# lucabaldesi/srsRAN

Hardware: AMD Instinct MI355X
Metric: PDSCH decoded Mbps + code-blocks/sec, 20 MHz TM4 QAM256, 1/2/4/8 GPU (higher is better)
Workload: dtype fp32+int16; 1 GPU; srslte_ue_dl chain from time-domain I/Q: 2048 subframes/GPU/batch, 20 MHz (100 PRB), TM4 2x2 spatial multiplexing, 2 codewords QAM256 TBS 97896 (C=16, K=6144), MMSE+CSI, max 10 half-its with CRC early stop, 40 dB crossed 2x2 channel, every subframe distinct (GPU eNodeB generator, keyed by global subframe index); 3 PHY worker threads (own ue_dl / stream / softbuffers each) decode alternate batches,; subframes_per_gpu_batch=2048, code_blocks_per_gpu_batch=65536, workers_per_gpu=3, parallelism=dp1

## Files before the change

### include/srsran_amd/dlsch.h

```cpp
#ifndef SRSRAN_AMD_DLSCH_H
#define SRSRAN_AMD_DLSCH_H

#include <stddef.h>
#include <stdint.h>

#ifdef __cplusplus
extern "C" {
#endif

typedef struct mi355_softbuffer_pool mi355_softbuffer_pool_t;

int  mi355_softbuffer_pool_create(mi355_softbuffer_pool_t** p, uint32_t nof_sb, uint32_t max_cb, int device);
void mi355_softbuffer_pool_destroy(mi355_softbuffer_pool_t* p);
int mi355_softbuffer_reset(mi355_softbuffer_pool_t* p, uint32_t sb, void* stream);
int mi355_softbuffer_reset_tbs(mi355_softbuffer_pool_t* p, uint32_t sb, uint32_t tbs, void* stream);
int mi355_softbuffer_reset_cb(mi355_softbuffer_pool_t* p, uint32_t sb, uint32_t nof_cb, void* stream);
int mi355_softbuffer_reset_all(mi355_softbuffer_pool_t* p, void* stream);
int mi355_softbuffer_reset_range(mi355_softbuffer_pool_t* p, uint32_t first, uint32_t n, void* stream);
int mi355_softbuffer_reset_tbs_batch(mi355_softbuffer_pool_t* p, const uint32_t* sbs, const uint32_t* tbs, uint32_t n,
                                     void* stream);
int mi355_softbuffer_pool_buffer(mi355_softbuffer_pool_t* p, int16_t** buf, uint32_t* stride, uint32_t* max_cb);
int mi355_softbuffer_pool_materialize(mi355_softbuffer_pool_t* p, uint32_t first, uint32_t n, void* stream);

int mi355_softbuffer_pool_data(mi355_softbuffer_pool_t* p, uint8_t** data, uint32_t* stride, uint32_t* nof_sb);
// ... 6 lines not shown
  uint32_t Qm;
  uint32_t rv;
  uint32_t softbuffer;
  uint64_t e_offset;
  uint64_t data_offset;
} mi355_dlsch_tb_t;

typedef struct mi355_dlsch mi355_dlsch_t;

int  mi355_dlsch_create(mi355_dlsch_t** q, int device);
void mi355_dlsch_destroy(mi355_dlsch_t* q);
int mi355_dlsch_set_max_iterations(mi355_dlsch_t* q, uint32_t max_iterations);
void mi355_dlsch_set_profiling(mi355_dlsch_t* q, int enable);

int mi355_dlsch_set_latency_path(int max_cbs);
int mi355_dlsch_latency_profile(int enable, uint64_t* out);
int  mi355_dlsch_kernel_stats(mi355_dlsch_t* q, double* ms, uint32_t* launches);

int mi355_dlsch_decode_dev(mi355_dlsch_t*           q,
                           mi355_softbuffer_pool_t* pool,
                           const int16_t*           d_e_bits,
                           const mi355_dlsch_tb_t*  tbs,
                           uint32_t                 ntb,
                           uint8_t*                 d_data,
                           int32_t*                 ret,
                           float*                   avg_iterations,
                           void*                    stream);

int mi355_dlsch_decode8_dev(mi355_dlsch_t* q, mi355_softbuffer_pool_t* pool, const int8_t* d_e_bits,
                            const mi355_dlsch_tb_t* tbs, uint32_t ntb, uint8_t* d_data, int32_t* ret,
// ... 7 lines not shown
```

### srsran_amd/csrc/dlsch_internal.h

```cpp
#pragma once
#include <hip/hip_runtime.h>
#include <stdint.h>

#define SB_STRIDE 18600
#define SB_DATA 768
#define SB_CONV8 10240
#define SB_ROWMASK 18544
#define SB_ROWMASK_WORDS 12

namespace mi355 {

struct CbDesc {
  uint32_t tb, cb, C;
  uint32_t rlen;
  uint32_t rp, n_e;
  uint32_t rv;
  uint32_t slot;
  uint64_t e_off;
  uint64_t data_off;
};

struct TbDesc {
  uint32_t tbs, C, C1, K1, K2, slot0, invalid;
  uint32_t Qm, nof_e_bits, rv;
  uint32_t cb_base[2];
  uint64_t e_off;
  uint64_t data_off;
  const uint32_t* crc_scale;
};

struct CrcTable {
  uint32_t t[256];
  uint32_t pw[24];
  uint32_t poly;
};

CrcTable make_crc_table(uint32_t poly);

constexpr uint16_t RM_NONE = 0xffff;

struct DlschRmArgs {
  const CbDesc*   desc;
  int             ncb;
  uint32_t        N;
  uint32_t        buflen;
  const uint16_t* inv[4];
  const int16_t*  e;
  int16_t*        sb;
  size_t          sb_stride;
  const uint8_t*  sb_crc;
  uint8_t*        fresh;
  uint32_t        fold2;
// ... 16 lines not shown
struct DlschCheckArgs {
  const CbDesc*  desc;
  int            ncb;
  uint32_t       K, h, max_its;
  const uint8_t* dec;
  size_t         dec_stride;
  uint8_t*       data;
  uint8_t*       done;
  const uint32_t* remaining;
  uint32_t*      next;
  uint32_t*      its;
  uint8_t*        sb_crc;
  const CrcTable* crc24a;
  const CrcTable* crc24b;
  const uint32_t* scale;
};

struct DlschTbArgs {
  const TbDesc* tb;
  int           ntb;
  uint8_t*      data;
  uint8_t*      sb_crc;
  uint8_t*      sb_data;
  int32_t*        ret;
  const CrcTable* crc24a;
  CbDesc*   desc;
  uint32_t* slot;
  uint32_t* its;
  uint8_t*  done;
  uint32_t* running;
  float*    avg;
};

struct DlschResetArgs {
  uint8_t* fresh;
  uint8_t* sb_crc;
  size_t   slot0, ncb;
  size_t   ncrc;
};

hipError_t dlsch_launch_rm(const DlschRmArgs& a, hipStream_t s);
hipError_t dlsch_launch_reset_list(const uint2* list, uint32_t n, uint32_t max_cb, uint8_t* fresh, uint8_t* cb_crc,
                                   hipStream_t s);
hipError_t dlsch_launch_check(const DlschCheckArgs& a, hipStream_t s);
hipError_t dlsch_launch_prologue(const DlschTbArgs& a, hipStream_t s);
hipError_t dlsch_launch_epilogue(const DlschTbArgs& a, hipStream_t s);
// ... 8 lines not shown
```

### srsran_amd/csrc/dlsch_kernels.hip

```cpp
#include <hip/hip_runtime.h>
#include <stdint.h>

#include "crc_device.h"
#include "dlsch_internal.h"
#include "rm_image.h"

namespace mi355 {

constexpr uint32_t RM_LDS     = 3 * 6144 + 12;
constexpr uint32_t RM_THREADS = 512;
constexpr int      RM_Q       = (3 * (6144 + 32) + 12 + 8 * RM_THREADS - 1) / (8 * RM_THREADS);
constexpr int      RM_EQ      = (RM_LDS + 8 * RM_THREADS - 1) / (8 * RM_THREADS);
#ifndef RM_CPB_N
#define RM_CPB_N 1
#endif
constexpr int      RM_CPB     = RM_CPB_N;

__device__ __forceinline__ uint32_t add_pairs(uint32_t a, uint32_t b)
{
  return ((a + b) & 0xffffu) | (((a >> 16) + (b >> 16)) << 16);
}

__device__ __forceinline__ uint4 ld_quad(const uint32_t* p, uint32_t q, uint32_t lim, bool al16, uint32_t fill)
{
// ... 174 lines not shown
    bool           todo  = false;
    if (lane < 3) data[tb.tbs / 8 + lane] = 0;
    for (uint32_t c = lane; c < tb.C; c += 64) {
      const uint32_t K    = c < tb.C1 ? tb.K1 : tb.K2;
      const uint32_t rlen = tb.C == 1 ? K : K - 24;
      uint32_t       rp = c * n_e, n_e2 = n_e;
      if (c > tb.C - gamma) {
        n_e2 = n_e + tb.Qm;
        rp   = (tb.C - gamma) * n_e + (c - (tb.C - gamma)) * n_e2;
      }
      const uint32_t g    = c < tb.C1 ? tb.cb_base[0] + c : tb.cb_base[1] + (c - tb.C1);
      const uint32_t slot = tb.slot0 + c;
      a.desc[g]           = CbDesc{(uint32_t)t, c, tb.C, rlen, rp, n_e2, tb.rv, slot, tb.e_off, tb.data_off};
      a.slot[g]           = slot;
      a.its[g]            = 0;
      const bool prior    = a.sb_crc[slot] != 0;
      a.done[g]           = prior ? 3 : 0;
      todo |= !prior;
    }
    if (todo) todo_any = 1;
    for (uint32_t c = 0; c < tb.C; c++) {
      const uint32_t slot = tb.slot0 + c;
      if (!a.sb_crc[slot]) continue;
      const uint32_t K    = c < tb.C1 ? tb.K1 : tb.K2;
      const uint32_t rlen = tb.C == 1 ? K : K - 24;
      const uint32_t o    = c * rlen / 8;
      for (uint32_t i = lane; i < rlen / 8; i += 64) data[o + i] = a.sb_data[(size_t)slot * 768 + i];
    }
  }
  __syncthreads();
  if (threadIdx.x == 0 && todo_any) flag_set(a.running);
}

__global__ __launch_bounds__(256) void dlsch_tb_epilogue(DlschTbArgs a)
{
  const int t   = blockIdx.x;
  const int tid = threadIdx.x;
  if (t >= a.ntb) return;
  __shared__ uint32_t t4[4][256];
  t4[0][tid] = a.crc24a->t[tid];
  __syncthreads();
  const TbDesc& tb = a.tb[t];
  if (tb.crc_scale) {
#pragma unroll
    for (int k = 1; k < 4; k++) {
      t4[k][tid] = crc24_step_table(t4[k - 1][tid], t4[0]);
      __syncthreads();
    }
  }
  if (tid == 0) {
    double sum = 0.0;
    for (uint32_t c = 0; c < tb.C; c++) sum += a.its[c < tb.C1 ? tb.cb_base[0] + c : tb.cb_base[1] + (c - tb.C1)];
    a.avg[t] = tb.C ? (float)(sum / tb.C) : 0.f;
  }
  if (tb.C == 0) {
    if (tid == 0) a.ret[t] = tb.invalid ? -2 : 0;
    return;
  }
  bool ok = true;
  for (uint32_t c = 0; c < tb.C; c++) ok &= a.sb_crc[tb.slot0 + c] != 0;
  uint8_t* data = a.data + tb.data_off;
  if (!ok) {
    for (uint32_t c = 0; c < tb.C; c++) {
      const uint32_t slot = tb.slot0 + c;
      if (!a.sb_crc[slot]) continue;
      const uint32_t K    = c < tb.C1 ? tb.K1 : tb.K2;
      const uint32_t rlen = tb.C == 1 ? K : K - 24;
      for (uint32_t i = tid; i < rlen / 8; i += blockDim.x) a.sb_data[(size_t)slot * 768 + i] = data[c * rlen / 8 + i];
    }
    if (tid == 0) a.ret[t] = -1;
    return;
  }
  const uint32_t par_rx = tb.crc_scale ? block_crc24_scaled4(data, tb.tbs / 8, t4, a.crc24a->poly, tb.crc_scale)
                                        : block_crc24(data, tb.tbs / 8, t4[0], *a.crc24a);
  if (tid == 0) {
    const uint32_t par_tx = ((uint32_t)data[tb.tbs / 8] << 16) | ((uint32_t)data[tb.tbs / 8 + 1] << 8) |
                            (uint32_t)data[tb.tbs / 8 + 2];
    a.ret[t] = (par_rx == par_tx && par_rx) ? 0 : -1;
  }
}

__global__ __launch_bounds__(256) void dlsch_sb_reset(DlschResetArgs a)
{
  const size_t g = (size_t)blockIdx.x * blockDim.x + threadIdx.x;
  if (g < a.ncb) a.fresh[a.slot0 + g] = 1;
  if (g < (a.ncrc ? a.ncrc : a.ncb)) a.sb_crc[a.slot0 + g] = 0;
}

__global__ __launch_bounds__(256) void dlsch_sb_reset_list(const uint2* list, uint32_t n, uint32_t max_cb, uint8_t* fresh,
                                                           uint8_t* cb_crc)
// ... 93 lines not shown
hipError_t dlsch_launch_check(const DlschCheckArgs& a, hipStream_t s)
{
  hipLaunchKernelGGL(dlsch_cb_check, dim3((unsigned)((a.ncb + 15) / 16)), dim3(1024), 0, s, a);
  return hipGetLastError();
}

hipError_t dlsch_launch_prologue(const DlschTbArgs& a, hipStream_t s)
{
  hipLaunchKernelGGL(dlsch_tb_prologue, dim3((unsigned)((a.ntb + 3) / 4)), dim3(256), 0, s, a);
  return hipGetLastError();
}

hipError_t dlsch_launch_epilogue(const DlschTbArgs& a, hipStream_t s)
{
  if (a.ntb <= 0) return hipSuccess;
  hipLaunchKernelGGL(dlsch_tb_epilogue, dim3((unsigned)a.ntb), dim3(256), 0, s, a);
  return hipGetLastError();
}

hipError_t dlsch_launch_reset(const DlschResetArgs& a, hipStream_t s)
{
  const size_t n = a.ncb > a.ncrc ? a.ncb : a.ncrc;
  if (!n) return hipSuccess;
  hipLaunchKernelGGL(dlsch_sb_reset, dim3((unsigned)((n + 255) / 256)), dim3(256), 0, s, a);
  return hipGetLastError();
}

}
```

### srsran_amd/csrc/dlsch_runtime.cpp

```cpp
#include <hip/hip_runtime.h>

#include <algorithm>
#include <chrono>
#include <stdlib.h>
#include <map>
#include <mutex>
#include <stdio.h>
#include <string.h>
#include <vector>

#include "../../include/srsran_amd/dlsch.h"
#include "../../include/srsran_amd/tdec.h"
#include "dlsch_internal.h"
#include "host_staging.h"
#include "tdec8_internal.h"
#include "rm_image.h"
#include "rm_tables.h"
#include "runtime_internal.h"
#include "tdec_internal.h"

using namespace mi355;

#define CHECK_HIP(x)                                                                                                   \
  do {                                                                                                                 \
// ... 48 lines not shown
struct mi355_dlsch {
  int                                    device = 0;
  hipStream_t                            own    = nullptr;
  uint32_t                               max_its = 10;
  std::map<uint32_t, mi355_tdec_batch_t*> dec;
  std::map<uint64_t, uint16_t*>          rm;
  std::map<uint64_t, uint16_t*>          rm8;
  struct Compact {
    uint16_t* d;
    uint32_t  nq, qoff;
  };
  std::map<uint64_t, Compact>            rmc;
  std::map<uint32_t, mi355_tdec8_t*>     dec8;
  std::map<uint32_t, uint32_t*>          scales;
  std::map<uint32_t, uint32_t*>          tb_scales;
  CrcTable*                              crc = nullptr;
  char*      scratch[2]     = {nullptr, nullptr};
  size_t     scratch_cap[2] = {0, 0};
  std::vector<void*> retired;
  hipEvent_t done_ev[2]     = {nullptr, nullptr};
  bool       done_armed[2]  = {false, false};
  uint32_t   par            = 0;
  std::mutex mu;
  bool       prof = false;
  HostStaging stage;
  HostStaging back;
  std::atomic<uint32_t> spec_mask{1u << 1};
};

static std::atomic<int> g_lat_cbs{-1};
// ... 26 lines not shown
  }
  return MI355_SUCCESS;
}

extern "C" int mi355_dlsch_set_latency_path(int max_cbs)
{
  const int old = lat_cbs_now();
  if (max_cbs >= 0) g_lat_cbs.store(max_cbs);
  return old;
}

static bool spec_enabled()
{
  static const bool on = !getenv("MI355_TDEC_SPEC") || atoi(getenv("MI355_TDEC_SPEC")) != 0;
  return on;
}

static bool no_rowmask()
{
  static const bool off = getenv("MI355_NO_ROWMASK") && atoi(getenv("MI355_NO_ROWMASK")) != 0;
  return off;
}

static bool lat_waves4()
{
  static const bool on = getenv("MI355_LAT_WAVES") && atoi(getenv("MI355_LAT_WAVES")) == 4;
  return on;
}
static bool lat_owaves()
{
// ... 59 lines not shown
static uint32_t gf2_mulmod24_host(uint32_t a, uint32_t b, uint32_t poly)
{
  uint32_t r = 0;
  for (int i = 23; i >= 0; i--) {
    r <<= 1;
    if (r & 0x1000000u) r ^= poly;
    if ((b >> i) & 1u) r ^= a;
  }
  return r & 0xffffffu;
}

static int crc_scales(mi355_dlsch_t* q, uint32_t K, const uint32_t** out)
{
  auto it = q->scales.find(K);
  if (it == q->scales.end()) {
    std::vector<uint32_t> t(144, 0u);
    const uint32_t        nbytes = K / 8, chunk = (nbytes + 63) / 64;
    const uint32_t        polys[2] = {0x1864CFB, 0x1800063};
    auto                  xpow = [](uint32_t after, uint32_t poly) {
      uint32_t sc = 1, x8 = 1u << 8;
      for (; after; after >>= 1) {
        if (after & 1) sc = gf2_mulmod24_host(sc, x8, poly);
        x8 = gf2_mulmod24_host(x8, x8, poly);
      }
      return sc;
    };
    const uint32_t nl = std::max(1u, mi355_tdec_autoimp_get_subblocks(K) / 2), cl = nbytes / nl;
    for (int pi = 0; pi < 2; pi++) {
      for (uint32_t lane = 0; lane < 64; lane++) {
        const uint32_t b0 = std::min(nbytes, lane * chunk), b1 = std::min(nbytes, b0 + chunk);
        t[pi * 64 + lane] = xpow(nbytes - b1, polys[pi]);
      }
      for (uint32_t l = 0; l < nl && l < 8; l++) t[128 + 8 * pi + l] = xpow(nbytes - (l + 1) * cl, polys[pi]);
    }
    uint32_t* d = nullptr;
    CHECK_HIP(hipMalloc(&d, t.size() * 4));
    CHECK_HIP(hipMemcpy(d, t.data(), t.size() * 4, hipMemcpyHostToDevice));
    it = q->scales.emplace(K, d).first;
  }
  *out = it->second;
  return MI355_SUCCESS;
}

static int tb_crc_scales(mi355_dlsch_t* q, uint32_t nbytes, const uint32_t** out)
{
  auto it = q->tb_scales.find(nbytes);
  if (it == q->tb_scales.end()) {
    std::vector<uint32_t> t(256);
    const uint32_t        chunk = ((nbytes + 255) / 256 + 3) / 4 * 4, poly = 0x1864CFB;
// ... 3 lines not shown
      for (uint32_t after = nbytes - b1; after; after >>= 1) {
        if (after & 1) sc = gf2_mulmod24_host(sc, x8, poly);
        x8 = gf2_mulmod24_host(x8, x8, poly);
      }
      t[tid] = sc;
    }
    uint32_t* d = nullptr;
    CHECK_HIP(hipMalloc(&d, t.size() * 4));
    CHECK_HIP(hipMemcpy(d, t.data(), t.size() * 4, hipMemcpyHostToDevice));
    it = q->tb_scales.emplace(nbytes, d).first;
  }
  *out = it->second;
  return MI355_SUCCESS;
}

static int scratch(mi355_dlsch_t* q, uint32_t k, size_t bytes, char** p)
{
  if (bytes > q->scratch_cap[k]) {
    if (q->scratch[k]) {
      q->retired.push_back(q->scratch[k]);
      q->scratch[k]    = nullptr;
      q->done_armed[k] = false;
    }
    size_t cap = bytes + bytes / 4 + 4096;
    CHECK_HIP(hipMalloc(&q->scratch[k], cap));
    q->scratch_cap[k] = cap;
  }
  *p = q->scratch[k];
  return MI355_SUCCESS;
}
// ... 187 lines not shown
  return MI355_SUCCESS;
}

void mi355_dlsch_destroy(mi355_dlsch_t* q)
{
  if (!q) return;
  (void)hipSetDevice(q->device);
  (void)hipDeviceSynchronize();
  for (auto& kv : q->dec) mi355_tdec_batch_destroy(kv.second);
  for (auto& kv : q->rm) (void)hipFree(kv.second);
  for (auto& kv : q->rm8) (void)hipFree(kv.second);
  for (auto& kv : q->rmc) (void)hipFree(kv.second.d);
  for (auto& kv : q->dec8) mi355_tdec8_destroy(kv.second);
  for (auto& kv : q->scales) (void)hipFree(kv.second);
  for (auto& kv : q->tb_scales) (void)hipFree(kv.second);
  (void)hipFree(q->crc);
  for (void* r : q->retired) (void)hipFree(r);
  for (int k = 0; k < 2; k++) {
    (void)hipFree(q->scratch[k]);
    if (q->done_ev[k]) (void)hipEventDestroy(q->done_ev[k]);
  }
  if (q->own) (void)hipStreamDestroy(q->own);
  delete q;
}

int mi355_dlsch_set_max_iterations(mi355_dlsch_t* q, uint32_t max_iterations)
{
  if (!q || max_iterations == 0) return MI355_ERROR_INVALID_INPUTS;
  q->max_its = max_iterations;
  return MI355_SUCCESS;
// ... 116 lines not shown
      if (j >= 32 * SB_ROWMASK_WORDS || j >= K / 16) return true;
      for (uint32_t w = 0; w < 16; w++)
        if (inv[s * sl + j * 16 + w] < E) return true;
      return false;
    };
    std::vector<uint16_t> rank(nquad, 0xffff);
    std::vector<uint32_t> qlist;
    for (uint32_t qd = 0; qd < nquad; qd++) {
      if (!defined(8 * qd)) continue;
      uint32_t m = 0;
      for (uint32_t p = 0; p < 8 && 8 * qd + p < buflen; p++) m |= (uint32_t)(inv[8 * qd + p] < E) << p;
      rank[qd] = (uint16_t)qlist.size();
      qlist.push_back(qd | m << 16);
    }
    const uint32_t        off = (E + 7) / 8 * 8;
    std::vector<uint16_t> all(off + 2 * qlist.size() + 8, 0);
    for (uint32_t r = 0; r < E; r++) {
      const uint32_t pos = t[r];
      if (rank[pos / 8] == 0xffff) return MI355_ERROR;
      all[r] = (uint16_t)(8 * rank[pos / 8] + pos % 8);
    }
    memcpy(all.data() + off, qlist.data(), qlist.size() * 4);
    uint16_t* d = nullptr;
    CHECK_HIP(hipMalloc(&d, all.size() * 2));
    CHECK_HIP(hipMemcpy(d, all.data(), all.size() * 2, hipMemcpyHostToDevice));
    CHECK_HIP(hipStreamSynchronize(nullptr));
    it = q->rmc.emplace(key, mi355_dlsch::Compact{d, (uint32_t)qlist.size(), off}).first;
  }
  *tab  = it->second.d;
  *nq   = it->second.nq;
  *qoff = it->second.qoff;
  return MI355_SUCCESS;
}

mi355::SoftbufferView mi355::softbuffer_view(mi355_softbuffer_pool_t* p)
{
  return SoftbufferView{p->buf, SB_STRIDE, p->cb_crc, p->fresh, p->nof_sb, p->max_cb};
}

int mi355::dlsch_decode_dev_hook(mi355_dlsch_t* q, mi355_softbuffer_pool_t* pool, const void* d_e_bits,
                                 const mi355_dlsch_tb_t* tbs, uint32_t ntb, uint8_t* d_data, int32_t* ret,
                                 float* avg_iterations, void* stream, mi355::WaitHook hook, bool llr8,
                                 mi355::DlschPending* pend, bool after_s, bool rm_done)
{
  if (!q || !pool || !tbs || !ret || (ntb && !d_e_bits)) return MI355_ERROR_INVALID_INPUTS;
  if (ntb == 0) return MI355_SUCCESS;
  std::lock_guard<std::mutex> lock(q->mu);
  static const bool prof = getenv("MI355_HOST_PROF") != nullptr;
  auto              now  = [] { return std::chrono::steady_clock::now(); };
  const auto        t0   = now();
  CHECK_HIP(hipSetDevice(q->device));
  hipStream_t s = stream ? (hipStream_t)stream : q->own;

  std::vector<TbDesc>                        tbd(ntb);
  std::vector<std::pair<uint32_t, uint32_t>> kcount;
  std::vector<uint32_t>                      rvmask;
  std::vector<uint32_t>                      fold2;
  auto group_of = [&](uint32_t K) {
    for (uint32_t i = 0; i < kcount.size(); i++)
      if (kcount[i].first == K) return i;
    kcount.push_back({K, 0u});
    rvmask.push_back(0u);
    return (uint32_t)kcount.size() - 1;
  };
  std::vector<uint8_t> grp(2 * ntb, 0);
  uint32_t             seg_tbs = UINT32_MAX;
  CbSegm               seg{};
// ... 11 lines not shown
    if (in.softbuffer >= pool->nof_sb || in.rv > 3 || in.Qm == 0 || seg_err) {
      d.invalid = 1;
      continue;
    }
    if (in.tbs == 0 || seg.C == 0) continue;
    if (seg.F || seg.C > pool->max_cb) {
      d.invalid = 1;
      continue;
    }
    auto ok8 = [](uint32_t K) { return tdec_subblocks_8bit(K) >= 16 || K <= 400; };
    if (llr8 && ((seg.C1 && !ok8(seg.K1)) || (seg.C > seg.C1 && !ok8(seg.K2)))) {
      d.invalid = 1;
      continue;
    }
    if (int e = tb_crc_scales(q, in.tbs / 8, &d.crc_scale)) return e;
    d.C          = seg.C;
    d.C1         = seg.C1;
    d.K1         = seg.K1;
    d.K2         = seg.K2;
    d.slot0      = in.softbuffer * pool->max_cb;
    d.Qm         = in.Qm;
    d.nof_e_bits = in.nof_e_bits;
    d.rv         = in.rv;
    d.e_off      = in.e_offset;
    const uint32_t emax = in.Qm * (in.nof_e_bits / in.Qm / seg.C + 1);
    auto           fold = [&](uint32_t g, uint32_t K) {
      if (fold2.size() <= g) fold2.resize(g + 1, 0);
      fold2[g] = std::max(fold2[g], std::min(emax, 3 * K + 12) / 2);
    };
    if (seg.C1) {
// ... 16 lines not shown
  std::vector<uint32_t> goff(kcount.size());
  size_t                total_cb = 0, dec_bytes = 0;
  for (size_t g = 0; g < kcount.size(); g++) {
    goff[g] = (uint32_t)total_cb;
    total_cb += kcount[g].second;
    dec_bytes += (size_t)kcount[g].second * (kcount[g].first / 8);
  }
  for (uint32_t t = 0; t < ntb; t++) {
    if (!tbd[t].C) continue;
    tbd[t].cb_base[0] += goff[grp[2 * t]];
    tbd[t].cb_base[1] += goff[grp[2 * t + 1]];
  }

  auto rnd = [](size_t b) { return (b + 255) / 256 * 256; };
  const size_t need = rnd(ntb * sizeof(TbDesc)) + rnd(4 * (q->max_its + 1)) + rnd(total_cb * sizeof(CbDesc)) +
                      3 * rnd(total_cb * 4) + rnd(total_cb) + rnd(dec_bytes) + 2 * rnd(ntb * 4);
  const uint32_t slot = q->par;
  q->par ^= 1u;
  char* base = nullptr;
  int   r    = scratch(q, slot, need, &base);
  if (r) return r;
  char* p     = base;
  auto  carve = [&](size_t b) {
    char* c = p;
    p += rnd(b);
    return c;
  };
  auto*        d_tb    = (TbDesc*)carve(ntb * sizeof(TbDesc));
  auto*        d_run   = (uint32_t*)carve(4 * (q->max_its + 1));
  const size_t staged  = (size_t)(p - base);
  auto*        d_cb    = (CbDesc*)carve(total_cb * sizeof(CbDesc));
  auto*        d_slot  = (uint32_t*)carve(total_cb * 4);
  auto*        d_its   = (uint32_t*)carve(total_cb * 4);
  auto*        d_done  = (uint8_t*)carve(total_cb);
  auto*        d_dec   = (uint8_t*)carve(dec_bytes);
  auto*        d_ret   = (int32_t*)carve(ntb * 4);
  auto*        d_avg   = (float*)carve(ntb * 4);

  CHECK_HIP(q->stage.reserve(staged));
  q->stage.put(tbd.data(), ntb * sizeof(TbDesc));
  q->stage.zeros(4 * (q->max_its + 1));
  CHECK_HIP(q->stage.upload(base, s, false, after_s && q->done_armed[slot] ? q->done_ev[slot] : nullptr));

  DlschTbArgs ta{d_tb,  (int)ntb, d_data, pool->cb_crc, pool->data, d_ret, &q->crc[0],
                 d_cb,  d_slot,   d_its,  d_done,       d_run,      d_avg};
  CHECK_HIP(dlsch_launch_prologue(ta, s));

  struct Live {
    uint32_t            K, off, n;
    uint8_t*            dec;
    mi355_tdec_batch_t* td;
    const uint32_t*     scale;
    mi355_tdec8_t*      t8 = nullptr;
  };
  std::vector<Live> live;
  size_t            off = 0, doff = 0;
  for (size_t gi = 0; gi < kcount.size(); gi++) {
    const uint32_t K = kcount[gi].first, n = kcount[gi].second;
    if (llr8) {
      const uint32_t nsb8 = tdec_subblocks_8bit(K);
// ... 94 lines not shown
  }
  const uint32_t spec_mask = spec_enabled() ? q->spec_mask.load() : 0u;
  for (uint32_t h = 0; h < q->max_its; h++) {
    const bool spec = h + 1 == q->max_its || ((spec_mask >> h) & 1u);
    for (size_t li = 0; li < live.size(); li++) {
      auto& lv = live[li];
      if (lat[li]) continue;
      if (lv.t8) {
        T8Batch b{};
        b.in = (int8_t*)pool->buf, b.in_stride = SB_STRIDE * sizeof(int16_t), b.slot = d_slot + lv.off;
        b.done = d_done + lv.off, b.running = d_run + h, b.K = lv.K, b.ncb = lv.n;
        if ((r = tdec8_halfit_batch(lv.t8, b, h, lv.dec, lv.K / 8, s))) return r;
      }
      DlschCheckArgs ca{d_cb + lv.off, (int)lv.n, lv.K, h, q->max_its, lv.dec, lv.K / 8, d_data,
                        d_done + lv.off, d_run + h, d_run + h + 1, d_its + lv.off, pool->cb_crc, &q->crc[0], &q->crc[1],
                        lv.scale};
      bool fused = false;
      if (!lv.t8) {
        TdecRun rq{llr8 ? pool->buf + SB_CONV8 : pool->buf, SB_STRIDE, d_slot + lv.off, d_done + lv.off, d_run + h, lv.n,
                   lv.K, h, h + 1, lv.dec, lv.K / 8, s, &ca, &fused};
        rq.rowmask = !llr8 && !no_rowmask();
        bool taken = false;
        rq.spec       = spec;
        rq.spec_taken = &taken;
        if ((r = mi355_tdec_run_internal(lv.td, rq))) return r;
        if (!fused) CHECK_HIP(dlsch_launch_check(ca, s));
        if (taken && h + 1 < q->max_its) {
          TdecRun rd = rq;
          rd.remaining  = d_run + h + 1;
          rd.chk        = nullptr;
          rd.chk_fused  = nullptr;
// ... 57 lines not shown
```

### srsran_amd/csrc/pdsch_internal.h

```cpp
#pragma once
#include <hip/hip_runtime.h>
#include <stdint.h>

namespace mi355 {

constexpr uint32_t EQ_BLOCK_ITEMS = 1024;

constexpr uint32_t PDSCH_GOLD_MAX = 14u * 12u * 110u * 8u;

struct PdschJobDev {
  const float2*   y[2];
  const float2*   h[4][2];
  const uint16_t* map;
  const uint16_t* imap;
  uint32_t        g0;
  float2*         d[2];
  float*          csi[2];
  uint32_t*       cmax;
  uint32_t        cmax_stride;
  uint32_t        nof_re, nof_rx, nof_ports, nof_layers, scheme, cb;
  uint32_t        row;
  uint32_t        row_magic;
  uint32_t        h_invariant;
  uint32_t        rhob_mask;
// ... 26 lines not shown

hipError_t pdsch_launch_equalize(const PdschJobDev* jobs, uint32_t njobs, uint32_t max_units, hipStream_t s);
hipError_t pdsch_launch_scr_pack(const uint32_t* c_init, uint32_t* const* dst, uint32_t n, const uint32_t* gold,
                                 uint32_t W, hipStream_t s);
hipError_t pdsch_launch_llr(const PdschCwDev* cws, uint32_t ncw, uint32_t max_pairs, hipStream_t s);
hipError_t pdsch_launch_fused(const PdschJobDev* jobs, uint32_t njobs, uint32_t max_pairs, const uint32_t* keys,
                              uint32_t nkeys, hipStream_t s);

struct EqRmLayer {
  const uint16_t* inv[2];
  uint32_t        N[2];
  uint32_t        buflen[2];
  uint32_t        C1;
  uint32_t        slot0;
};
struct EqRmJob {
  uint32_t  C, Qm, Gp;
  EqRmLayer layer[2];
  const uint16_t* cmp[2][2];
  uint32_t        cnq[2][2], cqoff[2][2];
};
struct EqRmPool {
  int16_t*       sb;
  size_t         sb_stride;
  const uint8_t* sb_crc;
  uint8_t*       fresh;
  int            sparse;
  int            diag = 0;
  unsigned long long* prof = nullptr;
};
hipError_t pdsch_launch_eq_rm(const PdschJobDev* jobs, const EqRmJob* rj, uint32_t njobs, uint32_t max_c, uint32_t img,
                              uint32_t cimg, const uint32_t* keys, uint32_t nkeys, const EqRmPool& pool, hipStream_t s);

// ... 2 lines not shown
```

### srsran_amd/csrc/pdsch_kernels.hip

```cpp
#include <hip/hip_runtime.h>

#include <algorithm>
#include <stdint.h>

#include "pdsch_internal.h"
#include "rm_image.h"
#include "xcd.h"

namespace mi355 {

namespace {

struct cf {
  float re, im;
};
__device__ __forceinline__ cf mk(float r, float i) { return cf{r, i}; }
__device__ __forceinline__ cf operator+(cf a, cf b) { return mk(a.re + b.re, a.im + b.im); }
__device__ __forceinline__ cf operator-(cf a, cf b) { return mk(a.re - b.re, a.im - b.im); }
__device__ __forceinline__ cf operator*(cf a, cf b) { return mk(a.re * b.re - a.im * b.im, a.re * b.im + a.im * b.re); }
__device__ __forceinline__ cf operator*(cf a, float s) { return mk(a.re * s, a.im * s); }
__device__ __forceinline__ cf cj(cf a) { return mk(a.re, -a.im); }
__device__ __forceinline__ cf mulj(cf a) { return mk(-a.im, a.re); }
__device__ __forceinline__ float abs2(cf a) { return a.re * a.re + a.im * a.im; }
#define GLB __attribute__((address_space(1)))
// ... 1085 lines not shown
  bool need[2], fresh[2];
  uint32_t slot[2];
#pragma unroll
  for (int l = 0; l < 2; l++) {
    slot[l]  = R.layer[l].slot0 + c;
    need[l]  = J.cw[l] != nullptr && !P.sb_crc[slot[l]];
    fresh[l] = need[l] && P.fresh[slot[l]] != 0;
  }
  if (!need[0] && !need[1]) return;
  const unsigned long long pt0 = P.prof ? clock64() : 0ull;
  const uint32_t      re0 = rp / Qm, re1 = (rp + n_e) / Qm, pairs = (J.nof_re + 1) / 2;
  const uint32_t      p1  = P.diag == 2 ? 0u : min((re1 + 1) / 2, pairs);
  const GLB uint32_t* map2  = (const GLB uint32_t*)gptr(J.map);
  const uint32_t      pb    = re0 / 2 + tid;
  uint32_t            mnext = pb < p1 ? map2[pb] : 0u;
  __shared__ uint32_t obm[2][2 * SB_ROWMASK_WORDS], nbm[2][2 * SB_ROWMASK_WORDS];
  if (tid < 2 * (2 * SB_ROWMASK_WORDS + 1)) {
    const uint32_t l = tid / (2 * SB_ROWMASK_WORDS + 1), w = tid % (2 * SB_ROWMASK_WORDS + 1);
    const uint32_t kx = c < R.layer[l].C1 ? 0u : 1u;
    if (need[l]) {
      uint32_t* bmg = rm_rowmask_of(P.sb + (size_t)slot[l] * P.sb_stride);
      if (w < 2 * SB_ROWMASK_WORDS) {
        const uint32_t nw = rm_rowmask_word(R.layer[l].inv[kx], R.layer[l].buflen[kx], fresh[l] ? n_e : 0x10000u, w);
        obm[l][w] = fresh[l] ? 0xffffffffu : bmg[w];
        nbm[l][w] = nw;
        bmg[w]    = nw;
      } else {
        bmg[w] = (R.layer[l].N[kx] - 12) / 3;
      }
    }
  }
  __shared__ PdschCwDev cwd[2];
  __shared__ uint32_t   cmb[2];
  static_assert(ER_THREADS >= 128 && 2 * (2 * SB_ROWMASK_WORDS + 1) <= 64, "pdsch_eq_rm prologue waves");
  if (tid - 64 < 2 && J.cw[tid - 64]) {
    const uint32_t l = tid - 64;
    cwd[l]           = *J.cw[l];
    cmb[l]           = cwd[l].csi_enable ? *gptr(cwd[l].cmax_final) : 0u;
  }
  __syncthreads();
  const uint32_t kx0 = c < R.layer[0].C1 ? 0u : 1u, kx1 = c < R.layer[1].C1 ? 0u : 1u;
  const bool     lean = need[0] && need[1] && fresh[0] && fresh[1] && R.layer[0].inv[kx0] == R.layer[1].inv[kx1] &&
                    R.layer[0].buflen[kx0] == R.layer[1].buflen[kx1];
  const uint32_t ev = c > R.C - gamma ? 1u : 0u;
  const bool     cm = lean && P.sparse && QM0 == QM1 && R.cmp[kx0][ev] != nullptr;
  const GLB uint16_t* fw  = cm ? gptr(R.cmp[kx0][ev]) : nullptr;
  const uint32_t      cnq = cm ? R.cnq[kx0][ev] : 0u;
  uint32_t* const     im32 = (uint32_t*)imgs;
  const unsigned long long pt1 = P.prof ? clock64() : 0ull;
  const float         noise = J.noise_dev ? *gptr(J.noise_dev) : J.noise;
  const uint32_t      row = J.row, magic = J.row_magic, rmask = J.rhob_mask;
  const float         rinv = J.rhob_inv;
  const GLB float2*   yp[2] = {gptr(J.y[0]), gptr(J.nof_rx > 1 ? J.y[1] : J.y[0])};
  const GLB float2*   hp[4];
  h_ptrs(J, hp);
  const GLB fv4*      wtp = (const GLB fv4*)gptr(J.wtab);
  uint4 iv0[ER_Q];
  if constexpr (ER_TPF) {
    if (lean) {
      const uint32_t  npairs = R.layer[0].buflen[kx0] / 2;
      const GLB uint32_t* inv32 = (const GLB uint32_t*)gptr(R.layer[0].inv[kx0]);
#pragma unroll
// ... 414 lines not shown
```

### srsran_amd/csrc/pdsch_runtime.cpp

```cpp
#include <hip/hip_runtime.h>

#include <algorithm>
#include <chrono>
#include <stdlib.h>
#include <cmath>
#include <map>
#include <unordered_map>
#include <atomic>
#include <mutex>
#include <stdio.h>
#include <string.h>
#include <string>
#include <vector>

#include "../../include/srsran_amd/dlsch.h"
#include "../../include/srsran_amd/pdsch.h"
#include "../../include/srsran_amd/tdec.h"
#include "host_staging.h"
#include "lte_common.h"
#include "pdsch_internal.h"
#include "rm_tables.h"
#include "runtime_internal.h"

using namespace mi355;
// ... 329 lines not shown
  D.noise      = cfg.decoder_type == MI355_MIMO_DECODER_ZF ? 0.0f : j.noise_estimate;
  D.units      = sch == MI355_TXSCHEME_DIVERSITY ? (np == 2 ? (nre + 1) / 2 : (nre + 3) / 4) : me.g1 - me.g0;
  for (uint32_t t = 0; t < 2; t++) {
    const mi355_ra_tb_t& tb = g.tb[t];
    P.decode[t]             = tb.enabled && !(res && res[t].crc);
    if (!P.decode[t]) continue;
    P.cw_of_tb[t] = tb.cw_idx;
    if (tb.cw_idx > 1 || mod_bits(tb.mod) == 0 || tb.nof_bits != nre * mod_bits(tb.mod) ||
        tb.nof_bits > PDSCH_GOLD_MAX || cfg.softbuffer[t] == UINT32_MAX || !j.payload[t])
      return MI355_ERROR_INVALID_INPUTS;
  }
  return MI355_SUCCESS;
}

static int run_frontend(mi355_pdsch_t* q, const mi355_pdsch_job_t* jobs, std::vector<JobPlan>& plans, hipStream_t s,
                        bool after_s = false, const EqRmPlan* er = nullptr)
{
  const auto     t_in  = std::chrono::steady_clock::now();
  const uint32_t njobs = (uint32_t)plans.size();
  size_t         nd = 0, ne = 0;
  std::vector<PdschCwDev> cws;
  std::vector<uint32_t>   new_ci;
  std::vector<uint32_t*>  new_dst;
  if (q->scr.size() > 4096) {
    CHECK_HIP(hipStreamSynchronize(s));
    for (auto& kv : q->scr) (void)hipFree(kv.second);
    q->scr.clear();
  }
  uint32_t  max_units = 0, max_pairs = 0, max_fpairs = 0;
  uint32_t  last_ci  = 0;
  const uint32_t* last_scr = nullptr;
// ... 105 lines not shown
      const uint32_t cw = plans[i].cw_of_tb[t];
      cws[ci].d         = plans[i].dev.d[cw];
      cws[ci].csi       = plans[i].dev.csi[cw];
      cws[ci].cmax      = plans[i].dev.cmax + (size_t)cw * nparts;
      cws[ci].nparts    = (plans[i].dev.units + EQ_BLOCK_ITEMS - 1) / EQ_BLOCK_ITEMS;
      cws[ci].cmax_final = d_cfin + ci;
      cws[ci].e         = q->e_arena + plans[i].e_off[t];
      if (q->llr8) {
        cws[ci].llr8  = 1;
        cws[ci].e8    = (int8_t*)q->e_arena + plans[i].e_off[t];
        cws[ci].k8[0] = (float)(-20 * M_SQRT2);
        cws[ci].k8[1] = 2 * 30 / sqrtf(10);
        cws[ci].k8[2] = 8.0f / sqrtf(170.0f);
        cws[ci].k8[3] = 4.0f / sqrtf(170.0f);
        cws[ci].k8[4] = 2.0f / sqrtf(170.0f);
      }
      ci++;
    }
  }
  static const bool prof = getenv("MI355_HOST_PROF") != nullptr;
  auto              now  = [] { return std::chrono::steady_clock::now(); };
  const auto        ta   = now();
  q->stage.put(hj.data(), njobs * sizeof(PdschJobDev));
  q->stage.put(cws.data(), ncw * sizeof(PdschCwDev));
  q->stage.put(new_ci.data(), new_ci.size() * 4);
  q->stage.put(new_dst.data(), new_dst.size() * 8);
  if (er) q->stage.put(er->rj.data(), njobs * sizeof(EqRmJob));
  const auto tb = now();
  CHECK_HIP(q->stage.upload(base, s, after_s, after_s && q->fe_armed ? q->fe_done : nullptr));
  const auto tc = now();
// ... 383 lines not shown
```

### srsran_amd/csrc/tdec_kernels.hip

```cpp
#include <hip/hip_runtime.h>

#include <atomic>
#include <stdint.h>
#include <stdlib.h>

#include "crc_device.h"
#include "tdec_internal.h"

namespace mi355 {

typedef short v2s __attribute__((ext_vector_type(2)));

__device__ __forceinline__ v2s U(uint32_t u) { return __builtin_bit_cast(v2s, u); }
__device__ __forceinline__ uint32_t W(v2s v) { return __builtin_bit_cast(uint32_t, v); }
__device__ __forceinline__ v2s sadd(v2s a, v2s b) { return __builtin_elementwise_add_sat(a, b); }
__device__ __forceinline__ v2s ssub(v2s a, v2s b) { return __builtin_elementwise_sub_sat(a, b); }
__device__ __forceinline__ v2s vmax(v2s a, v2s b) { return __builtin_elementwise_max(a, b); }
__device__ __forceinline__ v2s splat(short s) { return (v2s){s, s}; }
__device__ __forceinline__ uint32_t hi_lo(uint32_t a, uint32_t b) { return __builtin_amdgcn_alignbit(b, a, 16); }
__device__ __forceinline__ uint32_t from_prev(uint32_t v)
{
  return (uint32_t)__builtin_amdgcn_update_dpp(0, (int)v, 0x111, 0xf, 0xf, true);
}
__device__ __forceinline__ uint32_t from_next(uint32_t v)
// ... 98 lines not shown
    for (uint32_t i = tail0 + l; i < nb; i += NL) dst[i] = bytes[i];
    uint32_t* dw = (uint32_t*)(dst + head);
    const uint32_t sh = head;
    for (uint32_t w = l; w < nw; w += NL) {
      const uint32_t lo = bm[w + sh / 4], hi = bm[w + sh / 4 + 1];
      dw[w]             = sh ? __builtin_amdgcn_alignbyte(hi, lo, sh) : lo;
    }
    if (l == 0) {
      c.its[cb] = c.h + 1;
      if (ok) {
        c.done[cb]       = 1;
        c.sb_crc[d.slot] = 1;
      } else {
        c.done[cb] = 2;
      }
    }
  }
  const uint64_t un = __builtin_amdgcn_ballot_w64(l == 0 && !fin);
  if (un && (threadIdx.x & 63) == (uint32_t)__builtin_ctzll(un)) flag_set(c.next);
}


#define WG_AT(arr, j) (arr)[((size_t)grp * Lp + (j)) * 64 + q]

#define TDEC_BM_WORDS (8 * 193)
__shared__ uint32_t tdec_tx_lds[4][2][TDEC_SEG * 64];
__shared__ uint32_t tdec_ym_lds[4][8 * SB_ROWMASK_WORDS];
__shared__ uint32_t tdec_bm_lds[4 * TDEC_BM_WORDS];
__shared__ int16_t  tdec_stg_lds[4][TDEC_SEG * 128];
__shared__ uint32_t tdec_stg_row[4][TDEC_SEG];
// ... 792 lines not shown
```

Measured before the change: 129,800 Mbps.

## Compute TB CRC from per-code-block partial CRCs and pack epilogue four TBs per block

Each code block's CRC check now also computes a partial CRC24A over its payload bytes, scaled by a precomputed power of x, and stores it in a per-CB tb_part array. The TB epilogue then combines these partials with per-CB GF(2) scale factors instead of re-reading the whole transport block. When any partial is missing it falls back to a wave-parallel CRC. The epilogue now runs one wave per TB, four TBs per workgroup, and skips CRC table setup when partials suffice. Smaller changes precompute the rowmask bitmap on the host, move per-codeword data into the EqRm job, and skip the prologue restore loop when no CB was already decoded. These add work inside the decoder's check step and extra metadata.

```diff
diff --git a/include/srsran_amd/dlsch.h b/include/srsran_amd/dlsch.h
--- a/include/srsran_amd/dlsch.h
+++ b/include/srsran_amd/dlsch.h
@@ -44,6 +44,8 @@
 void mi355_dlsch_set_profiling(mi355_dlsch_t* q, int enable);
 
 int mi355_dlsch_set_latency_path(int max_cbs);
+
+int mi355_dlsch_set_tb_crc_parts(int on);
 int mi355_dlsch_latency_profile(int enable, uint64_t* out);
 int  mi355_dlsch_kernel_stats(mi355_dlsch_t* q, double* ms, uint32_t* launches);
 
diff --git a/srsran_amd/csrc/dlsch_internal.h b/srsran_amd/csrc/dlsch_internal.h
--- a/srsran_amd/csrc/dlsch_internal.h
+++ b/srsran_amd/csrc/dlsch_internal.h
@@ -27,6 +27,7 @@
   uint64_t e_off;
   uint64_t data_off;
   const uint32_t* crc_scale;
+  const uint32_t* part_scale;
 };
 
 struct CrcTable {
@@ -36,6 +37,8 @@
 };
 
 CrcTable make_crc_table(uint32_t poly);
+
+constexpr uint32_t TB_PART_VALID = 0x80000000u;
 
 constexpr uint16_t RM_NONE = 0xffff;
 
@@ -82,6 +85,7 @@
   const CrcTable* crc24a;
   const CrcTable* crc24b;
   const uint32_t* scale;
+  uint32_t* tb_part;
 };
 
 struct DlschTbArgs {
@@ -98,6 +102,7 @@
   uint8_t*  done;
   uint32_t* running;
   float*    avg;
+  uint32_t* tb_part;
 };
 
 struct DlschResetArgs {
diff --git a/srsran_amd/csrc/dlsch_kernels.hip b/srsran_amd/csrc/dlsch_kernels.hip
--- a/srsran_amd/csrc/dlsch_kernels.hip
+++ b/srsran_amd/csrc/dlsch_kernels.hip
@@ -212,12 +212,14 @@
       a.desc[g]           = CbDesc{(uint32_t)t, c, tb.C, rlen, rp, n_e2, tb.rv, slot, tb.e_off, tb.data_off};
       a.slot[g]           = slot;
       a.its[g]            = 0;
-      const bool prior    = a.sb_crc[slot] != 0;
+      if (a.tb_part) a.tb_part[g] = 0;
+      const bool prior   = a.sb_crc[slot] != 0;
       a.done[g]           = prior ? 3 : 0;
       todo |= !prior;
     }
     if (todo) todo_any = 1;
-    for (uint32_t c = 0; c < tb.C; c++) {
+    const bool restore = tb.C > 64 || __builtin_amdgcn_ballot_w64(todo) != (tb.C == 64 ? ~0ull : (1ull << tb.C) - 1);
+    for (uint32_t c = 0; restore && c < tb.C; c++) {
       const uint32_t slot = tb.slot0 + c;
       if (!a.sb_crc[slot]) continue;
       const uint32_t K    = c < tb.C1 ? tb.K1 : tb.K2;
@@ -230,48 +232,85 @@
   if (threadIdx.x == 0 && todo_any) flag_set(a.running);
 }
 
+__device__ __forceinline__ uint32_t wave_tb_crc24(const uint8_t* bytes, uint32_t nbytes, const uint32_t (*t4)[256],
+                                                  const CrcTable& T, const uint32_t* scale, uint32_t lane)
+{
+  const uint32_t chunk = 4 * (((nbytes + 255) / 256 + 3) / 4 * 4);
+  const uint32_t b0 = min(nbytes, lane * chunk), b1 = min(nbytes, b0 + chunk);
+  uint32_t       crc = crc24_words_any(bytes + b0, b1 - b0, t4);
+  uint32_t       sc  = 1;
+  if (scale) {
+    sc = scale[4 * lane + 3];
+  } else {
+    uint32_t after = nbytes - b1;
+    for (int i = 0; after; i++, after >>= 1) {
+      if (after & 1) sc = gf2_mulmod24(sc, T.pw[i], T.poly);
+    }
+  }
+  crc = gf2_mulmod24(crc, sc, T.poly);
+#pragma unroll
+  for (int o = 32; o >= 1; o >>= 1) crc ^= __shfl_xor(crc, o, 64);
+  return crc;
+}
+
 __global__ __launch_bounds__(256) void dlsch_tb_epilogue(DlschTbArgs a)
 {
-  const int t   = blockIdx.x;
-  const int tid = threadIdx.x;
-  if (t >= a.ntb) return;
+  const uint32_t tid = threadIdx.x, lane = tid & 63;
+  const int      t    = blockIdx.x * 4 + (int)(tid >> 6);
+  const bool     live = t < a.ntb;
+  const TbDesc&  tb   = a.tb[live ? t : 0];
+  const uint32_t C    = live ? tb.C : 0u;
+  const CrcTable& A   = *a.crc24a;
+  const bool     p0   = a.tb_part && tb.part_scale && C > 1;
+  bool           ok = true, pv = true;
+  uint32_t       its = 0, crc = 0;
+  for (uint32_t c = lane; c < C; c += 64) {
+    const uint32_t g = c < tb.C1 ? tb.cb_base[0] + c : tb.cb_base[1] + (c - tb.C1);
+    its += a.its[g];
+    ok &= a.sb_crc[tb.slot0 + c] != 0;
+    if (p0) {
+      const uint32_t p = a.tb_part[g];
+      pv &= a.done[g] == 1 && (p & TB_PART_VALID) != 0;
+      crc ^= gf2_mulmod24(p & 0xffffffu, tb.part_scale[c], A.poly);
+    }
+  }
+#pragma unroll
+  for (int o = 32; o >= 1; o >>= 1) {
+    its += __shfl_xor(its, o, 64);
+    crc ^= __shfl_xor(crc, o, 64);
+  }
+  ok = __builtin_amdgcn_ballot_w64(!ok) == 0;
+  const bool parts = p0 && __builtin_amdgcn_ballot_w64(!pv) == 0;
   __shared__ uint32_t t4[4][256];
-  t4[0][tid] = a.crc24a->t[tid];
-  __syncthreads();
-  const TbDesc& tb = a.tb[t];
-  if (tb.crc_scale) {
+  if (__syncthreads_or(C != 0 && ok && !parts)) {
+    t4[0][tid] = A.t[tid];
+    __syncthreads();
 #pragma unroll
     for (int k = 1; k < 4; k++) {
       t4[k][tid] = crc24_step_table(t4[k - 1][tid], t4[0]);
       __syncthreads();
     }
   }
-  if (tid == 0) {
-    double sum = 0.0;
-    for (uint32_t c = 0; c < tb.C; c++) sum += a.its[c < tb.C1 ? tb.cb_base[0] + c : tb.cb_base[1] + (c - tb.C1)];
-    a.avg[t] = tb.C ? (float)(sum / tb.C) : 0.f;
-  }
-  if (tb.C == 0) {
-    if (tid == 0) a.ret[t] = tb.invalid ? -2 : 0;
+  if (!live) return;
+  if (lane == 0) a.avg[t] = C ? (float)((double)its / C) : 0.f;
+  if (C == 0) {
+    if (lane == 0) a.ret[t] = tb.invalid ? -2 : 0;
     return;
   }
-  bool ok = true;
-  for (uint32_t c = 0; c < tb.C; c++) ok &= a.sb_crc[tb.slot0 + c] != 0;
   uint8_t* data = a.data + tb.data_off;
   if (!ok) {
-    for (uint32_t c = 0; c < tb.C; c++) {
+    for (uint32_t c = 0; c < C; c++) {
       const uint32_t slot = tb.slot0 + c;
       if (!a.sb_crc[slot]) continue;
       const uint32_t K    = c < tb.C1 ? tb.K1 : tb.K2;
-      const uint32_t rlen = tb.C == 1 ? K : K - 24;
-      for (uint32_t i = tid; i < rlen / 8; i += blockDim.x) a.sb_data[(size_t)slot * 768 + i] = data[c * rlen / 8 + i];
-    }
-    if (tid == 0) a.ret[t] = -1;
+      const uint32_t rlen = C == 1 ? K : K - 24;
+      for (uint32_t i = lane; i < rlen / 8; i += 64) a.sb_data[(size_t)slot * 768 + i] = data[c * rlen / 8 + i];
+    }
+    if (lane == 0) a.ret[t] = -1;
     return;
   }
-  const uint32_t par_rx = tb.crc_scale ? block_crc24_scaled4(data, tb.tbs / 8, t4, a.crc24a->poly, tb.crc_scale)
-                                        : block_crc24(data, tb.tbs / 8, t4[0], *a.crc24a);
-  if (tid == 0) {
+  const uint32_t par_rx = parts ? crc : wave_tb_crc24(data, tb.tbs / 8, t4, A, tb.crc_scale, lane);
+  if (lane == 0) {
     const uint32_t par_tx = ((uint32_t)data[tb.tbs / 8] << 16) | ((uint32_t)data[tb.tbs / 8 + 1] << 8) |
                             (uint32_t)data[tb.tbs / 8 + 2];
     a.ret[t] = (par_rx == par_tx && par_rx) ? 0 : -1;
@@ -395,7 +434,7 @@
 hipError_t dlsch_launch_epilogue(const DlschTbArgs& a, hipStream_t s)
 {
   if (a.ntb <= 0) return hipSuccess;
-  hipLaunchKernelGGL(dlsch_tb_epilogue, dim3((unsigned)a.ntb), dim3(256), 0, s, a);
+  hipLaunchKernelGGL(dlsch_tb_epilogue, dim3((unsigned)((a.ntb + 3) / 4)), dim3(256), 0, s, a);
   return hipGetLastError();
 }
 
diff --git a/srsran_amd/csrc/dlsch_runtime.cpp b/srsran_amd/csrc/dlsch_runtime.cpp
--- a/srsran_amd/csrc/dlsch_runtime.cpp
+++ b/srsran_amd/csrc/dlsch_runtime.cpp
@@ -86,6 +86,7 @@
   std::map<uint32_t, mi355_tdec8_t*>     dec8;
   std::map<uint32_t, uint32_t*>          scales;
   std::map<uint32_t, uint32_t*>          tb_scales;
+  std::map<uint32_t, uint32_t*>          tb_part_scales;
   CrcTable*                              crc = nullptr;
   char*      scratch[2]     = {nullptr, nullptr};
   size_t     scratch_cap[2] = {0, 0};
@@ -142,6 +143,24 @@
 {
   static const bool on = !getenv("MI355_TDEC_SPEC") || atoi(getenv("MI355_TDEC_SPEC")) != 0;
   return on;
+}
+
+static std::atomic<int> g_tb_crc_parts{-1};
+static bool             tb_crc_parts()
+{
+  int v = g_tb_crc_parts.load();
+  if (v < 0) {
+    v = !getenv("MI355_TB_CRC_PARTS") || atoi(getenv("MI355_TB_CRC_PARTS")) != 0;
+    g_tb_crc_parts.store(v);
+  }
+  return v != 0;
+}
+
+extern "C" int mi355_dlsch_set_tb_crc_parts(int on)
+{
+  const int old = tb_crc_parts() ? 1 : 0;
+  if (on >= 0) g_tb_crc_parts.store(on ? 1 : 0);
+  return old;
 }
 
 static bool no_rowmask()
@@ -231,7 +250,7 @@
 {
   auto it = q->scales.find(K);
   if (it == q->scales.end()) {
-    std::vector<uint32_t> t(144, 0u);
+    std::vector<uint32_t> t(160, 0u);
     const uint32_t        nbytes = K / 8, chunk = (nbytes + 63) / 64;
     const uint32_t        polys[2] = {0x1864CFB, 0x1800063};
     auto                  xpow = [](uint32_t after, uint32_t poly) {
@@ -250,6 +269,10 @@
       }
       for (uint32_t l = 0; l < nl && l < 8; l++) t[128 + 8 * pi + l] = xpow(nbytes - (l + 1) * cl, polys[pi]);
     }
+    for (uint32_t last = 0; last < 2 && nbytes >= 6; last++) {
+      const uint32_t nc = nbytes - 3 - 3 * last;
+      for (uint32_t l = 0; l < nl && l < 8; l++) t[144 + 8 * last + l] = xpow(nc - std::min(nc, (l + 1) * cl), polys[0]);
+    }
     uint32_t* d = nullptr;
     CHECK_HIP(hipMalloc(&d, t.size() * 4));
     CHECK_HIP(hipMemcpy(d, t.data(), t.size() * 4, hipMemcpyHostToDevice));
@@ -283,6 +306,29 @@
   return MI355_SUCCESS;
 }
 
+static int tb_part_scales(mi355_dlsch_t* q, uint32_t nbytes, uint32_t C, uint32_t K, const uint32_t** out)
+{
+  auto it = q->tb_part_scales.find(nbytes);
+  if (it == q->tb_part_scales.end()) {
+    std::vector<uint32_t> t(C);
+    const uint32_t        rb = K / 8 - 3, poly = 0x1864CFB;
+    for (uint32_t c = 0; c < C; c++) {
+      uint32_t sc = 1, x8 = 1u << 8;
+      for (uint32_t after = nbytes - std::min(nbytes, (c + 1) * rb); after; after >>= 1) {
+        if (after & 1) sc = gf2_mulmod24_host(sc, x8, poly);
+        x8 = gf2_mulmod24_host(x8, x8, poly);
+      }
+      t[c] = sc;
+    }
+    uint32_t* d = nullptr;
+    CHECK_HIP(hipMalloc(&d, t.size() * 4));
+    CHECK_HIP(hipMemcpy(d, t.data(), t.size() * 4, hipMemcpyHostToDevice));
+    it = q->tb_part_scales.emplace(nbytes, d).first;
+  }
+  *out = it->second;
+  return MI355_SUCCESS;
+}
+
 static int scratch(mi355_dlsch_t* q, uint32_t k, size_t bytes, char** p)
 {
   if (bytes > q->scratch_cap[k]) {
@@ -500,6 +546,7 @@
   for (auto& kv : q->dec8) mi355_tdec8_destroy(kv.second);
   for (auto& kv : q->scales) (void)hipFree(kv.second);
   for (auto& kv : q->tb_scales) (void)hipFree(kv.second);
+  for (auto& kv : q->tb_part_scales) (void)hipFree(kv.second);
   (void)hipFree(q->crc);
   for (void* r : q->retired) (void)hipFree(r);
   for (int k = 0; k < 2; k++) {
@@ -646,13 +693,27 @@
       qlist.push_back(qd | m << 16);
     }
     const uint32_t        off = (E + 7) / 8 * 8;
-    std::vector<uint16_t> all(off + 2 * qlist.size() + 8, 0);
+    uint32_t bm[2 * SB_ROWMASK_WORDS];
+    for (uint32_t w = 0; w < 2 * SB_ROWMASK_WORDS; w++) {
+      bm[w] = 0;
+      for (uint32_t b = 0; b < 32; b++) {
+        const uint32_t sj = 32 * w + b, st = sj / (32 * SB_ROWMASK_WORDS), j = sj % (32 * SB_ROWMASK_WORDS);
+        uint16_t       m  = 0;
+        if (tdec_subblocks(K) == 16 && j < K / 16) {
+          m = RM_NONE;
+          for (uint32_t x = 0; x < 16; x++) m = std::min(m, inv[(st + 1) * (K + 32) + j * 16 + x]);
+        }
+        bm[w] |= (uint32_t)(m < E) << b;
+      }
+    }
+    std::vector<uint16_t> all(off + 2 * qlist.size() + 4 * SB_ROWMASK_WORDS + 8, 0);
     for (uint32_t r = 0; r < E; r++) {
       const uint32_t pos = t[r];
       if (rank[pos / 8] == 0xffff) return MI355_ERROR;
       all[r] = (uint16_t)(8 * rank[pos / 8] + pos % 8);
     }
     memcpy(all.data() + off, qlist.data(), qlist.size() * 4);
+    memcpy(all.data() + off + 2 * qlist.size(), bm, sizeof(bm));
     uint16_t* d = nullptr;
     CHECK_HIP(hipMalloc(&d, all.size() * 2));
     CHECK_HIP(hipMemcpy(d, all.data(), all.size() * 2, hipMemcpyHostToDevice));
@@ -683,6 +744,7 @@
   const auto        t0   = now();
   CHECK_HIP(hipSetDevice(q->device));
   hipStream_t s = stream ? (hipStream_t)stream : q->own;
+  const bool  parts_on = tb_crc_parts();
 
   std::vector<TbDesc>                        tbd(ntb);
   std::vector<std::pair<uint32_t, uint32_t>> kcount;
@@ -724,6 +786,9 @@
       continue;
     }
     if (int e = tb_crc_scales(q, in.tbs / 8, &d.crc_scale)) return e;
+    if (seg.C > 1 && (seg.C1 == seg.C || seg.C1 == 0) && parts_on) {
+      if (int e = tb_part_scales(q, in.tbs / 8, seg.C, seg.C1 ? seg.K1 : seg.K2, &d.part_scale)) return e;
+    }
     d.C          = seg.C;
     d.C1         = seg.C1;
     d.K1         = seg.K1;
@@ -770,7 +835,7 @@
 
   auto rnd = [](size_t b) { return (b + 255) / 256 * 256; };
   const size_t need = rnd(ntb * sizeof(TbDesc)) + rnd(4 * (q->max_its + 1)) + rnd(total_cb * sizeof(CbDesc)) +
-                      3 * rnd(total_cb * 4) + rnd(total_cb) + rnd(dec_bytes) + 2 * rnd(ntb * 4);
+                      4 * rnd(total_cb * 4) + rnd(total_cb) + rnd(dec_bytes) + 2 * rnd(ntb * 4);
   const uint32_t slot = q->par;
   q->par ^= 1u;
   char* base = nullptr;
@@ -788,6 +853,7 @@
   auto*        d_cb    = (CbDesc*)carve(total_cb * sizeof(CbDesc));
   auto*        d_slot  = (uint32_t*)carve(total_cb * 4);
   auto*        d_its   = (uint32_t*)carve(total_cb * 4);
+  auto*        d_part  = (uint32_t*)carve(total_cb * 4);
   auto*        d_done  = (uint8_t*)carve(total_cb);
   auto*        d_dec   = (uint8_t*)carve(dec_bytes);
   auto*        d_ret   = (int32_t*)carve(ntb * 4);
@@ -799,7 +865,8 @@
   CHECK_HIP(q->stage.upload(base, s, false, after_s && q->done_armed[slot] ? q->done_ev[slot] : nullptr));
 
   DlschTbArgs ta{d_tb,  (int)ntb, d_data, pool->cb_crc, pool->data, d_ret, &q->crc[0],
-                 d_cb,  d_slot,   d_its,  d_done,       d_run,      d_avg};
+                 d_cb,  d_slot,   d_its,  d_done,       d_run,      d_avg,
+                 parts_on ? d_part : nullptr};
   CHECK_HIP(dlsch_launch_prologue(ta, s));
 
   struct Live {
@@ -924,7 +991,7 @@
       }
       DlschCheckArgs ca{d_cb + lv.off, (int)lv.n, lv.K, h, q->max_its, lv.dec, lv.K / 8, d_data,
                         d_done + lv.off, d_run + h, d_run + h + 1, d_its + lv.off, pool->cb_crc, &q->crc[0], &q->crc[1],
-                        lv.scale};
+                        lv.scale, parts_on ? d_part + lv.off : nullptr};
       bool fused = false;
       if (!lv.t8) {
         TdecRun rq{llr8 ? pool->buf + SB_CONV8 : pool->buf, SB_STRIDE, d_slot + lv.off, d_done + lv.off, d_run + h, lv.n,
diff --git a/srsran_amd/csrc/pdsch_internal.h b/srsran_amd/csrc/pdsch_internal.h
--- a/srsran_amd/csrc/pdsch_internal.h
+++ b/srsran_amd/csrc/pdsch_internal.h
@@ -64,9 +64,15 @@
   uint32_t        C1;
   uint32_t        slot0;
 };
+struct EqRmCw {
+  const uint32_t* scr;
+  const uint32_t* cmax_final;
+  uint32_t        nof_bits, nof_re, csi_enable;
+};
 struct EqRmJob {
   uint32_t  C, Qm, Gp;
   EqRmLayer layer[2];
+  EqRmCw    cw[2];
   const uint16_t* cmp[2][2];
   uint32_t        cnq[2][2], cqoff[2][2];
 };
diff --git a/srsran_amd/csrc/pdsch_kernels.hip b/srsran_amd/csrc/pdsch_kernels.hip
--- a/srsran_amd/csrc/pdsch_kernels.hip
+++ b/srsran_amd/csrc/pdsch_kernels.hip
@@ -1123,6 +1123,13 @@
   const GLB uint32_t* map2  = (const GLB uint32_t*)gptr(J.map);
   const uint32_t      pb    = re0 / 2 + tid;
   uint32_t            mnext = pb < p1 ? map2[pb] : 0u;
+  const uint32_t kx0 = c < R.layer[0].C1 ? 0u : 1u, kx1 = c < R.layer[1].C1 ? 0u : 1u;
+  const bool     lean = need[0] && need[1] && fresh[0] && fresh[1] && R.layer[0].inv[kx0] == R.layer[1].inv[kx1] &&
+                    R.layer[0].buflen[kx0] == R.layer[1].buflen[kx1];
+  const uint32_t ev = c > R.C - gamma ? 1u : 0u;
+  const bool     cm = lean && P.sparse && QM0 == QM1 && R.cmp[kx0][ev] != nullptr;
+  const GLB uint16_t* fw  = cm ? gptr(R.cmp[kx0][ev]) : nullptr;
+  const uint32_t      cnq = cm ? R.cnq[kx0][ev] : 0u;
   __shared__ uint32_t obm[2][2 * SB_ROWMASK_WORDS], nbm[2][2 * SB_ROWMASK_WORDS];
   if (tid < 2 * (2 * SB_ROWMASK_WORDS + 1)) {
     const uint32_t l = tid / (2 * SB_ROWMASK_WORDS + 1), w = tid % (2 * SB_ROWMASK_WORDS + 1);
@@ -1130,7 +1137,8 @@
     if (need[l]) {
       uint32_t* bmg = rm_rowmask_of(P.sb + (size_t)slot[l] * P.sb_stride);
       if (w < 2 * SB_ROWMASK_WORDS) {
-        const uint32_t nw = rm_rowmask_word(R.layer[l].inv[kx], R.layer[l].buflen[kx], fresh[l] ? n_e : 0x10000u, w);
+        const uint32_t nw = cm ? ((const GLB uint32_t*)(fw + R.cqoff[kx0][ev]))[cnq + w]
+                               : rm_rowmask_word(R.layer[l].inv[kx], R.layer[l].buflen[kx], fresh[l] ? n_e : 0x10000u, w);
         obm[l][w] = fresh[l] ? 0xffffffffu : bmg[w];
         nbm[l][w] = nw;
         bmg[w]    = nw;
@@ -1144,17 +1152,13 @@
   static_assert(ER_THREADS >= 128 && 2 * (2 * SB_ROWMASK_WORDS + 1) <= 64, "pdsch_eq_rm prologue waves");
   if (tid - 64 < 2 && J.cw[tid - 64]) {
     const uint32_t l = tid - 64;
-    cwd[l]           = *J.cw[l];
-    cmb[l]           = cwd[l].csi_enable ? *gptr(cwd[l].cmax_final) : 0u;
+    const EqRmCw&  w = R.cw[l];
+    PdschCwDev     d{};
+    d.scr = w.scr, d.nof_bits = w.nof_bits, d.nof_re = w.nof_re, d.csi_enable = w.csi_enable;
+    cwd[l] = d;
+    cmb[l] = w.csi_enable ? *gptr(w.cmax_final) : 0u;
   }
   __syncthreads();
-  const uint32_t kx0 = c < R.layer[0].C1 ? 0u : 1u, kx1 = c < R.layer[1].C1 ? 0u : 1u;
-  const bool     lean = need[0] && need[1] && fresh[0] && fresh[1] && R.layer[0].inv[kx0] == R.layer[1].inv[kx1] &&
-                    R.layer[0].buflen[kx0] == R.layer[1].buflen[kx1];
-  const uint32_t ev = c > R.C - gamma ? 1u : 0u;
-  const bool     cm = lean && P.sparse && QM0 == QM1 && R.cmp[kx0][ev] != nullptr;
-  const GLB uint16_t* fw  = cm ? gptr(R.cmp[kx0][ev]) : nullptr;
-  const uint32_t      cnq = cm ? R.cnq[kx0][ev] : 0u;
   uint32_t* const     im32 = (uint32_t*)imgs;
   const unsigned long long pt1 = P.prof ? clock64() : 0ull;
   const float         noise = J.noise_dev ? *gptr(J.noise_dev) : J.noise;
diff --git a/srsran_amd/csrc/pdsch_runtime.cpp b/srsran_amd/csrc/pdsch_runtime.cpp
--- a/srsran_amd/csrc/pdsch_runtime.cpp
+++ b/srsran_amd/csrc/pdsch_runtime.cpp
@@ -367,7 +367,7 @@
 }
 
 static int run_frontend(mi355_pdsch_t* q, const mi355_pdsch_job_t* jobs, std::vector<JobPlan>& plans, hipStream_t s,
-                        bool after_s = false, const EqRmPlan* er = nullptr)
+                        bool after_s = false, EqRmPlan* er = nullptr)
 {
   const auto     t_in  = std::chrono::steady_clock::now();
   const uint32_t njobs = (uint32_t)plans.size();
@@ -503,6 +503,14 @@
         cws[ci].k8[2] = 8.0f / sqrtf(170.0f);
         cws[ci].k8[3] = 4.0f / sqrtf(170.0f);
         cws[ci].k8[4] = 2.0f / sqrtf(170.0f);
+      }
+      if (er) {
+        EqRmCw& w    = er->rj[i].cw[cw & 1];
+        w.scr        = cws[ci].scr;
+        w.cmax_final = cws[ci].cmax_final;
+        w.nof_bits   = cws[ci].nof_bits;
+        w.nof_re     = cws[ci].nof_re;
+        w.csi_enable = cws[ci].csi_enable;
       }
       ci++;
     }
diff --git a/srsran_amd/csrc/tdec_kernels.hip b/srsran_amd/csrc/tdec_kernels.hip
--- a/srsran_amd/csrc/tdec_kernels.hip
+++ b/srsran_amd/csrc/tdec_kernels.hip
@@ -136,6 +136,16 @@
       } else {
         c.done[cb] = 2;
       }
+    }
+    if (ok && pi && c.tb_part) {
+      const uint32_t last = d.cb + 1 == d.C ? 1u : 0u;
+      const uint32_t nc   = d.rlen / 8 - 3 * last;
+      const uint32_t b0 = min(nc, l * chunk), b1 = min(nc, (l + 1) * chunk);
+      uint32_t       p  = crc24_words(bytes + b0, b1 - b0, t4[0]);
+      p                 = gf2_mulmod24(p, c.scale[144 + 8 * last + l], c.crc24a->poly);
+#pragma unroll
+      for (int o = NL / 2; o >= 1; o >>= 1) p ^= (uint32_t)__shfl_xor((int)p, o, 64);
+      if (l == 0) c.tb_part[cb] = TB_PART_VALID | p;
     }
   }
   const uint64_t un = __builtin_amdgcn_ballot_w64(l == 0 && !fin);
```

After: 130,800 Mbps, median of 3. About the same (+0.7%).
